# firstBusiness/mathmap

Hardware: AMD Instinct MI355X
Metric: Mpixels/sec (mandelbrot @8192x8192) (higher is better)
Workload: dtype f32

## Files before the change

### mathmap_amd/csrc/hipgen_internal.h

```cpp
#pragma once
#include <functional>
#include <memory>
#include <optional>
#include <ostream>
#include <string>
#include <vector>

#include "hipgen.h"

namespace mm {
namespace hipgen {

enum Slice { PROLOGUE, PIXEL, ROWS };

std::optional<int> env_int(const char *name);
struct Knobs {
    std::optional<int> unroll = env_int("MMHIP_UNROLL");
    std::optional<int> tile_w = env_int("MMHIP_TILE_W");
    std::optional<int> single_pixel = env_int("MMHIP_SINGLE_PIXEL");
    std::optional<int> pair = env_int("MMHIP_PAIR");
    bool pair_debug = env_int("MMHIP_PAIR_DEBUG").has_value();
    std::optional<int> pair_masks = env_int("MMHIP_PAIR_MASKS");
    std::optional<int> pair_exit = env_int("MMHIP_PAIR_EXIT");
    std::optional<int> pair_exit_tail = env_int("MMHIP_PAIR_EXIT_TAIL");
    std::optional<int> pair_pack = env_int("MMHIP_PAIR_PACK");
    std::optional<int> pair_peel = env_int("MMHIP_PAIR_PEEL");
    std::optional<int> pair_fma2 = env_int("MMHIP_PAIR_FMA2");
    bool pair_no_uniform = env_int("MMHIP_PAIR_NO_UNIFORM").has_value();
    std::optional<int> nt_store = env_int("MMHIP_NT_STORE");
    std::optional<int> xcd_order = env_int("MMHIP_XCD_ORDER");
    std::optional<int> waves_per_eu = env_int("MMHIP_WAVES_PER_EU");
    bool no_fetched_result = env_int("MMHIP_NO_FETCHED_RESULT").has_value();
    bool no_same_taps = env_int("MMHIP_NO_SAME_TAPS").has_value();
    bool no_outside_shortcut = env_int("MMHIP_NO_OUTSIDE_SHORTCUT").has_value();
    std::optional<int> frame_hot = env_int("MMHIP_FRAME_HOT");
    bool no_row_slice = env_int("MMHIP_NO_ROW_SLICE").has_value();
    std::optional<int> max_call_depth = env_int("MMHIP_MAX_CALL_DEPTH");
};

std::string vname(const Value *v);
std::string ctype(const CompVar *v);
int type_size(const CompVar *v);
std::string float_literal(float f);
const char *libm_name(const char *cname, bool f32);
bool is_truth_op(const char *cname);
bool is_pow2_divisor(float c);
bool nonneg_or_nan(const Value *v, int depth);
const Primary *sqrt_less_pow2(const Rhs &r, float *kk);

struct PairEnv {
    std::ostream &out;
    FilterCode &code;
    const KernelOptions &opt;
    const Knobs &knobs;
    const std::vector<Value *> &pix_defs;
    int pixel_stmts, pixel_fetches;
    std::function<std::string(const Primary &)> prim;
    std::function<std::string(const Stmt *)> rhs;
    std::function<bool(const Value *)> value_visible;
};
struct PairMode {
    virtual ~PairMode() {}
    virtual bool exit_driven() const = 0;
    virtual bool is_uniform(const Value *v) const = 0;
    virtual void emit_helpers() = 0;
    virtual void emit_pixel_loop(const std::string &ind) = 0;
};
std::unique_ptr<PairMode> make_pair_mode(const PairEnv &env);

}
}
```

### mathmap_amd/csrc/hipgen_pair.cpp

```cpp
#include <algorithm>
#include <cstdio>
#include <cstring>
#include <map>
#include <set>

#include "hipgen_internal.h"

namespace mm {
namespace hipgen {
namespace {

struct PairGen final : PairMode {
    PairEnv env;
    std::ostream &out;
    FilterCode &code;
    std::set<const Value *> defs;
    std::set<const Value *> bools;
    std::set<const Value *> uniform;
    int ids = 0;
    const bool exit = env.knobs.pair_exit.value_or(1) && env.knobs.pair_masks.value_or(1);
    const bool pack = exit && env.knobs.pair_pack.value_or(1);
    const Stmt *split_def = nullptr;
    bool split_leave = false;
    const bool fma2 = exit && env.knobs.pair_fma2.value_or(1) && env.knobs.pair_exit_tail.value_or(2) >= 2;
    struct Fuse { const Stmt *r, *d; Primary t, b; float k; bool keep_d; };
    std::map<const Stmt *, std::vector<Fuse>> fuse_plan;
    std::map<const Stmt *, const Fuse *> fusing;
    std::set<const Stmt *> fused_away;

    explicit PairGen(const PairEnv &e) : env(e), out(e.out), code(e.code) {}

    bool exit_driven() const override { return exit; }
    bool is_uniform(const Value *v) const override { return uniform.count(v) > 0; }

    static bool scalar_ty(Ty t) { return t == Ty::Int || t == Ty::Float; }
    static bool prim_ok(const Primary &p) {
        if (p.kind == Primary::IntConst || p.kind == Primary::FloatConst) return true;
        return p.kind == Primary::Val && scalar_ty(p.value->var->type);
    }
    static bool rhs_ok(const Rhs &r) {
        if (r.kind == Rhs::Prim) return prim_ok(r.prim);
        if (r.kind == Rhs::Internal) return r.internal == "x" || r.internal == "y";
        if (r.kind != Rhs::Op) return false;
        static const char *ok[] = {"ADD", "SUB", "MUL", "NEG", "DIV", "LESS", "LEQ", "EQ", "NOT", "sqrt"};
        bool found = false;
        for (const char *o : ok) found = found || !strcmp(r.op->cname, o);
        if (!found) return false;
        for (const Primary &a : r.args) if (!prim_ok(a)) return false;
        if (!strcmp(r.op->cname, "sqrt") && r.args[0].type() != Ty::Float) return false;
        if (!strcmp(r.op->cname, "NOT") && r.args[0].type() != Ty::Int) return false;
        return true;
    }
    bool block_ok(const Block &b) const {
        for (const Stmt *s : b) {
            if (!s->in_pixel) continue;
            switch (s->kind) {
                case Stmt::Assign:
                    if (!s->lhs || !scalar_ty(s->lhs->var->type) || !rhs_ok(s->rhs)) {
                        if (env.knobs.pair_debug)
                            fprintf(stderr, "pair mode: statement not covered (%s)\n",
                                    s->rhs.kind == Rhs::Op ? s->rhs.op->cname : s->rhs.kind == Rhs::Internal ? s->rhs.internal.c_str() : "rhs kind");
                        return false;
                    }
                    break;
                case Stmt::If:
                case Stmt::While:
                    if (s->cond.kind != Rhs::Prim || !prim_ok(s->cond.prim) || s->cond.prim.type() != Ty::Int) return false;
                    for (const Stmt *ph : s->phis) {
                        if (!ph->in_pixel) continue;
                        if (!scalar_ty(ph->lhs->var->type) || ph->rhs.kind != Rhs::Prim || ph->rhs2.kind != Rhs::Prim ||
                            !prim_ok(ph->rhs.prim) || !prim_ok(ph->rhs2.prim))
                            return false;
                    }
                    if (s->kind == Stmt::If ? !(block_ok(s->then_) && block_ok(s->else_)) : !block_ok(s->body)) return false;
                    break;
                default: break;
            }
        }
        return true;
    }
    bool eligible() const {
        if (!env.opt.fast_math_exact) return false;
        const bool force = env.knobs.pair.has_value();
        if (force && !*env.knobs.pair) return false;
        const int stmts = env.pixel_stmts;
        if (env.pixel_fetches || stmts < 4 || stmts > (force ? 400 : 40)) return false;
        const bool dbg = env.knobs.pair_debug;
        for (int i = 0; i < 4; ++i)
            if (!code.result[i] || !scalar_ty(code.result[i]->var->type)) {
                if (dbg) fprintf(stderr, "pair mode: result %d is not an int / float value\n", i);
                return false;
            }
        const bool ok = block_ok(code.body);
        if (dbg) fprintf(stderr, "pair mode: body %s (%d statements)\n", ok ? "covered" : "not covered", stmts);
        return ok;
    }

    template <class P> static bool truth_def(const Stmt *d, P operand) {
        if (d->kind == Stmt::Phi) return d->rhs.kind == Rhs::Prim && d->rhs2.kind == Rhs::Prim && operand(d->rhs.prim) && operand(d->rhs2.prim);
        if (d->kind != Stmt::Assign) return false;
        if (d->rhs.kind == Rhs::Prim) return operand(d->rhs.prim);
        return d->rhs.kind == Rhs::Op && is_truth_op(d->rhs.op->cname);
    }
    static bool const_is_bool(const Value *v, int depth) {
        if (!v || depth > 12 || v->var->type != Ty::Int) return false;
        if (v->index < 0) return true;
        return v->def && truth_def(v->def, [&](const Primary &p) {
            return p.kind == Primary::IntConst ? p.i == 0 || p.i == 1 : p.kind == Primary::Val && const_is_bool(p.value, depth + 1);
        });
    }
    bool prim_bool(const Primary &p) const {
        if (p.kind == Primary::IntConst) return p.i == 0 || p.i == 1;
        if (p.kind != Primary::Val) return false;
        if (p.value->index < 0) return p.value->var->type == Ty::Int;
        if (bools.count(p.value)) return true;
        return !defs.count(p.value) && const_is_bool(p.value, 0);
    }
    void infer_bools() {
        std::vector<const Stmt *> idefs;
        for (Value *v : env.pix_defs) {
            defs.insert(v);
            if (v->var->type == Ty::Int && v->def && v->def->lhs == v) idefs.push_back(v->def);
        }
        for (const Stmt *d : idefs) bools.insert(d->lhs);
        for (bool changed = true; changed;) {
            changed = false;
            for (const Stmt *d : idefs)
                if (bools.count(d->lhs) && !truth_def(d, [&](const Primary &p) { return prim_bool(p); })) { bools.erase(d->lhs); changed = true; }
        }
    }
    void uses_outside(const Block &b, const Stmt *skip, std::set<const Value *> &uses) const {
        auto use = [&](const Primary &p) { if (p.kind == Primary::Val) uses.insert(p.value); };
        auto use_rhs = [&](const Rhs &r) { if (r.kind == Rhs::Prim) use(r.prim); for (const Primary &a : r.args) use(a); };
        for (const Stmt *s : b) {
            if (!s->in_pixel) continue;
            if (s->kind == Stmt::Assign) use_rhs(s->rhs);
            if (s->kind == Stmt::If) {
                use_rhs(s->cond);
                uses_outside(s->then_, skip, uses);
                uses_outside(s->else_, skip, uses);
                for (const Stmt *ph : s->phis) if (ph->in_pixel) { use_rhs(ph->rhs); use_rhs(ph->rhs2); }
            }
            if (s->kind == Stmt::While) {
                for (const Stmt *ph : s->phis) if (ph->in_pixel) { use_rhs(ph->rhs); if (s != skip) use_rhs(ph->rhs2); }
                if (s != skip) { use_rhs(s->cond); uses_outside(s->body, skip, uses); }
            }
        }
    }

    std::string pbool(const Primary &p) {
        const std::string bu = exit ? "mm_xbu(" : "mm_bu(";
        if (p.kind == Primary::IntConst) return bu + (p.i ? "true)" : "false)");
        if (p.kind == Primary::Val && p.value->index < 0) return bu + "false)";
        if (uniform.count(p.value)) return "mm_bu((bool)u" + vname(p.value) + ")";
        if (bools.count(p.value)) return vname(p.value);
        return "mm_tob(" + pprim(p, Ty::Int) + ")";
    }
    std::string pprim(const Primary &p, Ty want) {
        const char *w = want == Ty::Float ? "mm_vf(" : "mm_vi(";
        if (p.kind == Primary::IntConst) return std::string(w) + std::to_string(p.i) + ")";
        if (p.kind == Primary::FloatConst) return std::string(w) + float_literal(p.f) + "f)";
        if (p.value->index < 0) return std::string(w) + "0)";
        if (uniform.count(p.value))
            return std::string(w) + (p.value->var->type == Ty::Float ? "(float)u" : "(int)u") + vname(p.value) + ")";
        return std::string(w) + vname(p.value) + ")";
    }
    static Ty arith_ty(const Rhs &r) {
        for (const Primary &a : r.args) if (a.type() == Ty::Float) return Ty::Float;
        return Ty::Int;
    }
    std::string prhs(const Rhs &r, const Value *lhs) {
        const Ty lhs_ty = lhs->var->type;
        const bool as_bool = bools.count(lhs) > 0;
        if (r.kind == Rhs::Prim) return as_bool ? pbool(r.prim) : pprim(r.prim, lhs_ty);
        if (r.kind == Rhs::Internal) return r.internal == "x" ? "mm_vf(x)" : "mm_y2";
        const char *cn = r.op->cname;
        const Ty t = arith_ty(r);
        const char *op = !strcmp(cn, "ADD") ? "+" : !strcmp(cn, "SUB") ? "-" : !strcmp(cn, "MUL") ? "*" : !strcmp(cn, "LESS") ? "<"
                         : !strcmp(cn, "LEQ") ? "<=" : !strcmp(cn, "EQ") ? "==" : nullptr;
        const bool compares = op && (op[0] == '<' || op[0] == '=');
        if (op && r.args.size() == 2 && ((r.args[0].type() == Ty::Int && r.args[1].kind == Primary::FloatConst) ||
                                         (r.args[1].type() == Ty::Int && r.args[0].kind == Primary::FloatConst))) {
            auto comp = [&](const Primary &p, const char *c) {
                if (p.kind == Primary::FloatConst) return "(double)" + float_literal(p.f) + "f";
                return "(double)" + pprim(p, Ty::Int) + "." + c;
            };
            const std::string ex = comp(r.args[0], "x") + " " + op + " " + comp(r.args[1], "x");
            const std::string ey = comp(r.args[0], "y") + " " + op + " " + comp(r.args[1], "y");
            if (compares) {
                const std::string b = "mm_bl(" + ex + ", " + ey + ")";
                return as_bool ? b : "mm_vi(" + b + ")";
            }
            return "mm_pf{(float)(" + ex + "), (float)(" + ey + ")}";
        }
        if (op && !compares) return "(" + pprim(r.args[0], t) + " " + op + " " + pprim(r.args[1], t) + ")";
        if (!strcmp(cn, "NEG")) return "(-" + pprim(r.args[0], t) + ")";
        if (!strcmp(cn, "sqrt")) return "mm_sqrt2(" + pprim(r.args[0], Ty::Float) + ")";
        if (!strcmp(cn, "DIV")) {
            if (r.args[1].kind == Primary::FloatConst || r.args[1].kind == Primary::IntConst) {
                const float c = r.args[1].kind == Primary::FloatConst ? r.args[1].f : (float)r.args[1].i;
                if (is_pow2_divisor(c)) return "(" + pprim(r.args[0], Ty::Float) + " * " + float_literal(1.0f / c) + "f)";
            }
            return "(" + pprim(r.args[0], Ty::Float) + " / " + pprim(r.args[1], Ty::Float) + ")";
        }
        std::string b;
        const std::string notb = exit ? "mm_xnotb(" : "mm_notb(";
        if (!strcmp(cn, "NOT")) b = notb + pbool(r.args[0]) + ")";
        else if (!strcmp(cn, "EQ") && prim_bool(r.args[0]) && prim_bool(r.args[1])) {
            const Primary &x = r.args[0], &y = r.args[1];
            if (y.kind == Primary::IntConst) b = y.i ? pbool(x) : notb + pbool(x) + ")";
            else if (x.kind == Primary::IntConst) b = x.i ? pbool(y) : notb + pbool(y) + ")";
            else b = "mm_eqb(" + pbool(x) + ", " + pbool(y) + ")";
        } else {
            float kk = 0;
            const Primary *sq = sqrt_less_pow2(r, &kk);
            if (sq && env.value_visible(sq->value)) {
                const std::string a = pprim(*sq, Ty::Float), k2 = "mm_vf(" + float_literal(kk) + "f)";
                b = nonneg_or_nan(sq->value, 0) ? "mm_lt(" + a + ", " + k2 + ")"
                                                : "mm_andb(mm_lt(" + a + ", " + k2 + "), mm_le(mm_vf(0.0f), " + a + "))";
            } else {
                const char *fn = !strcmp(cn, "LESS") ? "mm_lt(" : !strcmp(cn, "LEQ") ? "mm_le(" : "mm_eq(";
                b = fn + pprim(r.args[0], t) + ", " + pprim(r.args[1], t) + ")";
            }
        }
        return as_bool ? b : "mm_vi(" + b + ")";
    }
    std::string pair_ctype(const Value *v) const {
        return bools.count(v) ? "mm_bb" : v->var->type == Ty::Float ? "mm_pf" : "mm_pi";
    }
    std::string pval_as(const Primary &p, const Value *lhs) {
        return bools.count(lhs) ? pbool(p) : pprim(p, lhs->var->type);
    }

    bool invariant_scalar(const Primary &p) const {
        if (p.kind == Primary::IntConst || p.kind == Primary::FloatConst) return true;
        if (p.kind != Primary::Val) return false;
        return p.value->index < 0 || !defs.count(p.value);
    }
    bool uniform_operand(const Primary &p) const {
        return invariant_scalar(p) || (p.kind == Primary::Val && uniform.count(p.value));
    }
    void mark_uniform(const Block &b) {
        for (const Stmt *s : b) {
            if (!s->in_pixel) continue;
            if (s->kind == Stmt::Assign && s->rhs.kind != Rhs::Internal) {
                bool ok = s->rhs.kind == Rhs::Prim ? uniform_operand(s->rhs.prim) : s->rhs.kind == Rhs::Op;
                if (ok && s->rhs.kind == Rhs::Op)
                    for (const Primary &a : s->rhs.args) ok = ok && uniform_operand(a);
                if (ok && s->rhs.kind == Rhs::Prim && !(s->rhs.prim.kind == Primary::Val && uniform.count(s->rhs.prim.value))) ok = false;
                if (ok && bools.count(s->lhs) && !exit) ok = false;
                if (ok) uniform.insert(s->lhs);
            } else if (s->kind == Stmt::If) {
                mark_uniform(s->then_);
                mark_uniform(s->else_);
            }
        }
    }
    std::vector<const Stmt *> find_uniform_ivs(const Stmt *w) {
        std::vector<const Stmt *> ivs;
        if (env.knobs.pair_no_uniform) return ivs;
        for (const Stmt *ph : w->phis) {
            if (!ph->in_pixel || ph->rhs.kind != Rhs::Prim || ph->rhs2.kind != Rhs::Prim) continue;
            if (!scalar_ty(ph->lhs->var->type) || bools.count(ph->lhs)) continue;
            if (!invariant_scalar(ph->rhs.prim) || ph->rhs2.prim.kind != Primary::Val) continue;
            const Stmt *d = ph->rhs2.prim.value->def;
            if (!d || d->kind != Stmt::Assign || d->parent != w || d->rhs.kind != Rhs::Op || d->rhs.args.size() != 2) continue;
            const char *cn = d->rhs.op->cname;
            const Primary &a0 = d->rhs.args[0], &a1 = d->rhs.args[1];
            const bool self0 = a0.kind == Primary::Val && a0.value == ph->lhs, self1 = a1.kind == Primary::Val && a1.value == ph->lhs;
            const bool step = (!strcmp(cn, "ADD") && ((self0 && invariant_scalar(a1)) || (self1 && invariant_scalar(a0)))) ||
                              (!strcmp(cn, "SUB") && self0 && invariant_scalar(a1));
            if (!step) continue;
            ivs.push_back(ph);
            uniform.insert(ph->lhs);
        }
        if (!ivs.empty()) mark_uniform(w->body);
        return ivs;
    }

    struct Body {
        std::set<const Value *> defs;
        std::map<const Value *, const Stmt *> if_of;
        std::vector<const Stmt *> order;
        bool nested_loop = false;
    };
    void scan_body(const Block &b, Body &pb) const {
        for (const Stmt *s : b) {
            if (!s->in_pixel) continue;
            if (s->kind == Stmt::Assign) { pb.defs.insert(s->lhs); pb.order.push_back(s); }
            if (s->kind == Stmt::While) pb.nested_loop = true;
            if (s->kind == Stmt::If) {
                scan_body(s->then_, pb);
                scan_body(s->else_, pb);
                for (const Stmt *ph : s->phis)
                    if (ph->in_pixel) { pb.defs.insert(ph->lhs); pb.if_of[ph->lhs] = s; pb.order.push_back(ph); }
            }
        }
    }
    int eval3(const Primary &p, const Body &pb, const Value *l, int lv, int depth = 0) const {
        if (p.kind == Primary::IntConst) return p.i == 0 ? 0 : p.i == 1 ? 1 : -1;
        if (p.kind != Primary::Val || depth > 32) return -1;
        if (p.value->index < 0) return 0;
        if (p.value == l) return lv;
        if (!pb.defs.count(p.value) || !bools.count(p.value)) return -1;
        const Stmt *d = p.value->def;
        if (!d) return -1;
        if (d->kind == Stmt::Phi) {
            auto it = pb.if_of.find(p.value);
            if (it == pb.if_of.end() || d->rhs.kind != Rhs::Prim || d->rhs2.kind != Rhs::Prim) return -1;
            const Primary &cp = it->second->cond.prim;
            const int c = eval3(cp, pb, l, lv, depth + 1);
            const bool same1 = cp.kind == Primary::Val && d->rhs.prim.kind == Primary::Val && d->rhs.prim.value == cp.value && bools.count(cp.value);
            const bool same2 = cp.kind == Primary::Val && d->rhs2.prim.kind == Primary::Val && d->rhs2.prim.value == cp.value && bools.count(cp.value);
            const int a = same1 ? 1 : eval3(d->rhs.prim, pb, l, lv, depth + 1);
            const int b = same2 ? 0 : eval3(d->rhs2.prim, pb, l, lv, depth + 1);
            if (c == 1) return a;
            if (c == 0) return b;
            return a == b ? a : -1;
        }
        if (d->kind != Stmt::Assign) return -1;
        if (d->rhs.kind == Rhs::Prim) return eval3(d->rhs.prim, pb, l, lv, depth + 1);
        if (d->rhs.kind != Rhs::Op) return -1;
        const char *cn = d->rhs.op->cname;
        if (!strcmp(cn, "NOT")) { const int x = eval3(d->rhs.args[0], pb, l, lv, depth + 1); return x < 0 ? -1 : !x; }
        if (!strcmp(cn, "EQ") && prim_bool(d->rhs.args[0]) && prim_bool(d->rhs.args[1])) {
            const int x = eval3(d->rhs.args[0], pb, l, lv, depth + 1), y = eval3(d->rhs.args[1], pb, l, lv, depth + 1);
            return x < 0 || y < 0 ? -1 : x == y;
        }
        return -1;
    }
    const Stmt *find_split(const Stmt *w, const std::set<const Value *> &outside, bool &leave) const {
        if (w->cond.prim.kind != Primary::Val) return nullptr;
        Body pb;
        scan_body(w->body, pb);
        if (pb.nested_loop) return nullptr;
        const Stmt *cph = nullptr;
        for (const Stmt *ph : w->phis) if (ph->in_pixel && ph->lhs == w->cond.prim.value) cph = ph;
        if (!cph || cph->rhs2.kind != Rhs::Prim) return nullptr;
        for (const Stmt *d : pb.order) {
            if (d->kind != Stmt::Assign || !uniform.count(d->lhs) || !bools.count(d->lhs) || d->rhs.kind != Rhs::Op) continue;
            if (!is_truth_op(d->rhs.op->cname) || d->rhs.args.size() != 2) continue;
            if (d->rhs.args[0].type() != Ty::Int || d->rhs.args[1].type() != Ty::Int) continue;
            for (int lv = 0; lv < 2; ++lv) {
                if (eval3(cph->rhs2.prim, pb, d->lhs, lv) != 0) continue;
                std::set<const Value *> dep{d->lhs};
                auto in = [&](const Primary &p) { return p.kind == Primary::Val && dep.count(p.value) > 0; };
                for (const Stmt *q : pb.order) {
                    bool dp = false;
                    if (q->kind == Stmt::Assign) { if (q->rhs.kind == Rhs::Prim) dp = in(q->rhs.prim); for (const Primary &a : q->rhs.args) dp = dp || in(a); }
                    else dp = in(pb.if_of.at(q->lhs)->cond.prim) || in(q->rhs.prim) || in(q->rhs2.prim);
                    if (dp) dep.insert(q->lhs);
                }
                bool ok = true;
                for (const Stmt *ph : w->phis)
                    if (ph->in_pixel && outside.count(ph->lhs) && in(ph->rhs2.prim)) ok = false;
                if (!ok) continue;
                leave = lv != 0;
                return d;
            }
        }
        return nullptr;
    }
    bool tail_operand(const Primary &p, std::string &text, std::vector<std::string> &inputs, int first_input) {
        if (p.kind == Primary::IntConst) { text = std::to_string(p.i); return true; }
        if (p.kind != Primary::Val) return false;
        text = "%" + std::to_string(first_input + (int)inputs.size());
        inputs.push_back("__builtin_amdgcn_readfirstlane((int)(" + env.prim(p) + "))");
        return true;
    }

    struct Loop {
        Stmt *s;
        std::string ind, a;
        std::set<const Value *> outside;
        std::vector<const Stmt *> ivs;
        std::vector<std::pair<const Stmt *, std::string>> exit_copy;
        bool counted = false;
        unsigned count_step = 0;
        const Stmt *count_iv = nullptr;
        std::string count_twin;
        bool is_iv(const Stmt *ph) const { return std::find(ivs.begin(), ivs.end(), ph) != ivs.end(); }
    };
    void step_phis(const Loop &w, const std::string &I, bool select) {
        std::vector<Stmt *> phis;
        for (Stmt *ph : w.s->phis) if (ph->in_pixel && (select || !w.is_iv(ph))) phis.push_back(ph);
        for (size_t k = 0; k < phis.size(); ++k) {
            const std::string nv = pval_as(phis[k]->rhs2.prim, phis[k]->lhs);
            out << I << "const " << pair_ctype(phis[k]->lhs) << " " << w.a << "_n" << k << " = "
                << (select && w.outside.count(phis[k]->lhs) ? "mm_sel2(" + w.a + ", " + nv + ", " + vname(phis[k]->lhs) + ")" : nv) << ";\n";
        }
        for (size_t k = 0; k < phis.size(); ++k) out << I << vname(phis[k]->lhs) << " = " << w.a << "_n" << k << ";\n";
        for (const Stmt *ph : w.ivs)
            if (ph != w.count_iv) out << I << "u" << vname(ph->lhs) << " = " << env.prim(ph->rhs2.prim) << ";\n";
    }
    static bool counted_relation(const char *cn, bool leave, int side, long step, bool &inclusive) {
        if (!strcmp(cn, "EQ")) { inclusive = false; return leave && (step == 1 || step == -1); }
        const bool advancing_left = leave ? side == 1 : side == 0;
        inclusive = leave ? !strcmp(cn, "LESS") : !strcmp(cn, "LEQ");
        return advancing_left ? step > 0 : step < 0;
    }
    void plan_counted(Loop &w, const std::string &l) {
        if (env.knobs.pair_exit_tail.value_or(2) < 2) return;
        bool leave = false;
        const Stmt *split = find_split(w.s, w.outside, leave);
        if (!split) return;
        const char *cn = split->rhs.op->cname;
        const bool eq = !strcmp(cn, "EQ");
        int side = -1;
        const Stmt *iv = nullptr;
        long step = 0;
        bool stepped = false;
        for (int i = 0; i < 2 && side < 0; ++i) {
            const Primary &p = split->rhs.args[i];
            if (p.kind != Primary::Val) continue;
            for (const Stmt *ph : w.ivs) {
                if (ph->lhs->var->type != Ty::Int) continue;
                const Stmt *d = ph->rhs2.prim.value->def;
                const bool self0 = d->rhs.args[0].kind == Primary::Val && d->rhs.args[0].value == ph->lhs;
                const Primary &c = d->rhs.args[self0 ? 1 : 0];
                if (c.kind != Primary::IntConst || (p.value != ph->lhs && p.value != d->lhs)) continue;
                side = i; iv = ph; stepped = p.value == d->lhs;
                step = !strcmp(d->rhs.op->cname, "SUB") ? -(long)c.i : (long)c.i;
            }
        }
        if (side < 0 || step == 0 || step > 0x7fffffffL || step < -0x7fffffffL) return;
        const Primary &bound = split->rhs.args[1 - side], &init = iv->rhs.prim;
        if (!invariant_scalar(bound) || bound.type() != Ty::Int || init.type() != Ty::Int) return;
        bool inclusive = false;
        if (!counted_relation(cn, leave, side, step, inclusive)) return;
        const bool up = step > 0;
        const long pre = stepped ? 0 : -step;
        auto lit = [](const Primary &p, long &v) {
            if (p.kind == Primary::IntConst) { v = p.i; return true; }
            if (p.kind == Primary::Val && p.value->index < 0) { v = 0; return true; }
            return false;
        };
        long iv0 = 0, b0 = 0;
        const std::string k = l + "_k";
        if (lit(init, iv0) && lit(bound, b0)) {
            long d = up ? b0 - (iv0 + pre) : (iv0 + pre) - b0;
            if (eq) d &= 0xffffffffL; else d += inclusive ? 1 : 0;
            if (!eq && d > 0xffffffffL) return;
            const bool exact = eq || d > 0;
            if (!exact) d = 1;
            const unsigned k0 = 0u - (unsigned)d;
            out << w.ind << "unsigned " << k << " = " << k0 << "u;\n";
            if (exact) {
                w.count_iv = iv;
                const unsigned c = up ? (unsigned)iv0 - k0 : (unsigned)iv0 + k0;
                w.count_twin = "(int)(" + std::to_string(c) + "u " + (up ? "+ " : "- ") + k + ")";
            }
        } else {
            uniform.erase(iv->lhs);
            const std::string o = "((long)(" + env.prim(init) + ") + " + std::to_string(pre) + "l)", b = "(long)(" + env.prim(bound) + ")";
            uniform.insert(iv->lhs);
            const std::string d = (up ? b + " - " + o : o + " - " + b) + (inclusive ? " + 1l" : "");
            out << w.ind << "const long " << k << "_d = " << d << ";\n";
            out << w.ind << "unsigned " << k << " = __builtin_amdgcn_readfirstlane(0u - (unsigned)("
                << (eq ? k + "_d" : k + "_d <= 0l ? 1l : " + k + "_d > 0xffffffffl ? 0xffffffffl : " + k + "_d") << "));\n";
        }
        w.counted = true;
        w.count_step = (unsigned)(up ? step : -step);
    }
    void selecting_iteration(const Loop &w) {
        Stmt *s = w.s;
        const std::string &ind = w.ind, &a = w.a;
        stmts(s->body, ind + "  ", a);
        step_phis(w, ind + "  ", true);
        out << ind << "  " << a << " = mm_andb(" << a << ", " << pbool(s->cond.prim) << ");\n";
    }
    void exit_driven_iteration(const Loop &w, const std::string &l) {
        Stmt *s = w.s;
        const std::string &ind = w.ind, &a = w.a, I2 = ind + "    ";
        bool leave = false;
        const Stmt *split = find_split(s, w.outside, leave);
        std::vector<std::string> tail_inputs;
        std::string tail_o0, tail_o1;
        const bool asm_tail = split && !w.counted && env.knobs.pair_exit_tail.value_or(1) &&
                              !(split->rhs.args[0].kind == Primary::IntConst && split->rhs.args[1].kind == Primary::IntConst) &&
                              tail_operand(split->rhs.args[0], tail_o0, tail_inputs, 8) && tail_operand(split->rhs.args[1], tail_o1, tail_inputs, 8);
        out << ind << "  mm_bb " << l << ";"
            << (w.counted ? " unsigned long " + l + "_t;" : asm_tail ? " unsigned long " + l + "_u, " + l + "_t;" : split ? " bool " + l + "_b;" : "") << "\n";
        out << ind << "  do {\n";
        if (w.count_iv) out << I2 << "const int u" << vname(w.count_iv->lhs) << " = " << w.count_twin << ";\n";
        const Stmt *outer_split = split_def;
        const bool outer_leave = split_leave;
        split_def = split;
        split_leave = leave;
        stmts(s->body, I2, a);
        split_def = outer_split;
        split_leave = outer_leave;
        if (asm_tail)
            for (size_t i = 0; i < tail_inputs.size(); ++i) {
                out << I2 << "const int " << l << "_o" << i << " = " << tail_inputs[i] << ";\n";
                tail_inputs[i] = l + "_o" + std::to_string(i);
            }
        else if (split && !w.counted)
            out << I2 << l << "_b = (bool)(" << env.rhs(split) << ") == " << (leave ? "true" : "false") << ";\n";
        step_phis(w, I2, false);
        const std::string c = pbool(s->cond.prim);
        const std::string lx = a + ".x & ~" + c + ".x", ly = a + ".y & ~" + c + ".y";
        if (w.counted) {
            out << I2 << "const mm_bb " << l << "_c = " << c << ";\n";
            out << I2 << "asm(\"s_andn2_b64 %0, %4, %6\\n\\ts_andn2_b64 %1, %5, %7\\n\\ts_or_b64 %3, %0, %1\\n\\ts_add_u32 %2, %2, " << w.count_step
                << "\\n\\ts_cselect_b64 %3, -1, %3\"\n"
                << I2 << "    : \"=&s\"(" << l << ".x), \"=&s\"(" << l << ".y), \"+s\"(" << l << "_k), \"=&s\"(" << l << "_t)\n"
                << I2 << "    : \"s\"(" << a << ".x), \"s\"(" << a << ".y), \"s\"(" << l << "_c.x), \"s\"(" << l << "_c.y) : \"scc\");\n";
            out << ind << "  } while (" << l << "_t == 0);\n";
            out << ind << "  if (" << l << "_k < " << w.count_step << "u) " << l << " = " << a << ";      // the counter has wrapped: every active lane leaves\n";
            if (w.count_iv) out << ind << "  u" << vname(w.count_iv->lhs) << " = " << w.count_twin << ";\n";
        } else if (asm_tail) {
            const char *cn = split->rhs.op->cname;
            const char *cmp = !strcmp(cn, "LESS") ? "s_cmp_lt_i32" : !strcmp(cn, "LEQ") ? "s_cmp_le_i32" : "s_cmp_eq_i32";
            out << I2 << "const mm_bb " << l << "_c = " << c << ";\n";
            out << I2 << "asm(\"" << cmp << " " << tail_o0 << ", " << tail_o1 << "\\n\\ts_cselect_b64 %2, " << (leave ? "-1, 0" : "0, -1")
                << "\\n\\ts_andn2_b64 %0, %4, %6\\n\\ts_andn2_b64 %1, %5, %7\\n\\ts_or_b64 %3, %2, %0\\n\\ts_or_b64 %3, %3, %1\"\n"
                << I2 << "    : \"=&s\"(" << l << ".x), \"=&s\"(" << l << ".y), \"=&s\"(" << l << "_u), \"=&s\"(" << l << "_t)\n"
                << I2 << "    : \"s\"(" << a << ".x), \"s\"(" << a << ".y), \"s\"(" << l << "_c.x), \"s\"(" << l << "_c.y)";
            for (const std::string &in : tail_inputs) out << ", \"s\"(" << in << ")";
            out << " : \"scc\");\n";
            out << ind << "  } while (" << l << "_t == 0);\n";
            out << ind << "  " << l << ".x |= " << a << ".x & " << l << "_u; " << l << ".y |= " << a << ".y & " << l << "_u;\n";
        } else if (split) {
            out << I2 << l << " = mm_bb{" << lx << ", " << ly << "};\n";
            out << ind << "  } while (!" << l << "_b && (" << l << ".x | " << l << ".y) == 0);\n";
            out << ind << "  if (" << l << "_b) " << l << " = " << a << ";      // the uniform conjunct has ended the loop: every active lane leaves\n";
        } else {
            out << I2 << l << " = mm_bb{" << lx << ", " << ly << "};\n";
            out << ind << "  } while ((" << l << ".x | " << l << ".y) == 0);\n";
        }
        for (const auto &e : w.exit_copy) {
            std::string nv = vname(e.first->lhs);
            if (w.is_iv(e.first)) nv = e.first->lhs->var->type == Ty::Float ? "mm_vf((float)u" + nv + ")" : "mm_vi(mm_s2v((int)u" + nv + "))";
            out << ind << "  " << e.second << " = mm_sel2(" << l << ", " << nv << ", " << e.second << ");\n";
        }
        out << ind << "  " << a << ".x &= ~" << l << ".x; " << a << ".y &= ~" << l << ".y;\n";
    }
    struct Uses { std::map<const Value *, int> live, dead; };
    template <class F> static void each_phi(const Block &b, F f) {
        for (const Stmt *s : b) {
            for (const Stmt *ph : s->phis) f(ph);
            each_phi(s->then_, f);
            each_phi(s->else_, f);
            each_phi(s->body, f);
        }
    }
    static void count_roots(const Block &b, std::map<const Value *, int> &n) {
        auto use = [&](const Primary &p) { if (p.kind == Primary::Val) ++n[p.value]; };
        auto use_rhs = [&](const Rhs &r) { if (r.kind == Rhs::Prim) use(r.prim); for (const Primary &a : r.args) use(a); };
        for (const Stmt *s : b) {
            if (s->kind == Stmt::Assign) use_rhs(s->rhs);
            if (s->kind == Stmt::If || s->kind == Stmt::While) use_rhs(s->cond);
            count_roots(s->then_, n);
            count_roots(s->else_, n);
            count_roots(s->body, n);
        }
    }
    Uses count_uses() const {
        Uses u;
        count_roots(code.body, u.live);
        for (int i = 0; i < 4; ++i) if (code.result[i]) ++u.live[code.result[i]];
        std::vector<const Stmt *> phis;
        each_phi(code.body, [&](const Stmt *ph) { phis.push_back(ph); });
        std::set<const Stmt *> live_phis;
        auto operands = [](const Stmt *ph, auto f) {
            for (const Rhs *r : {&ph->rhs, &ph->rhs2}) if (r->kind == Rhs::Prim && r->prim.kind == Primary::Val) f(r->prim.value);
        };
        for (bool changed = true; changed;) {
            changed = false;
            for (const Stmt *ph : phis)
                if (!live_phis.count(ph) && u.live.count(ph->lhs)) {
                    live_phis.insert(ph);
                    operands(ph, [&](const Value *v) { ++u.live[v]; });
                    changed = true;
                }
        }
        for (const Stmt *ph : phis)
            if (!live_phis.count(ph)) operands(ph, [&](const Value *v) { ++u.dead[v]; });
        return u;
    }
    static void defined_in(const Block &b, std::set<const Value *> &d) {
        for (const Stmt *s : b) {
            if (s->kind == Stmt::Assign) d.insert(s->lhs);
            for (const Stmt *ph : s->phis) d.insert(ph->lhs);
            defined_in(s->then_, d);
            defined_in(s->else_, d);
            defined_in(s->body, d);
        }
    }
    static int count_stmts(const Block &b) {
        int n = 0;
        for (const Stmt *s : b)
            if (s->in_pixel) n += 1 + count_stmts(s->then_) + count_stmts(s->else_) + count_stmts(s->body);
        return n;
    }
    static bool pow2_multiplier(const Primary &p, float &k) {
        if (p.kind != Primary::IntConst && p.kind != Primary::FloatConst) return false;
        k = p.kind == Primary::IntConst ? (float)p.i : p.f;
        if (!(k >= 2.0f) || k > 0x1p127f) return false;
        unsigned bits;
        memcpy(&bits, &k, 4);
        return (bits & 0x7fffffu) == 0;
    }
    static bool doubling(const Stmt *d, Primary &t, float &k) {
        if (d->kind != Stmt::Assign || !d->in_pixel || d->lhs->var->type != Ty::Float || d->rhs.kind != Rhs::Op || d->rhs.args.size() != 2) return false;
        const Primary &a0 = d->rhs.args[0], &a1 = d->rhs.args[1];
        auto fval = [](const Primary &p) { return p.kind == Primary::Val && p.value->var->type == Ty::Float; };
        if (!strcmp(d->rhs.op->cname, "ADD") && fval(a0) && fval(a1) && a0.value == a1.value) { t = a0; k = 2.0f; return true; }
        if (strcmp(d->rhs.op->cname, "MUL")) return false;
        if (fval(a0) && pow2_multiplier(a1, k)) { t = a0; return true; }
        if (fval(a1) && pow2_multiplier(a0, k)) { t = a1; return true; }
        return false;
    }
    void plan_block(const Block &b, const std::set<const Value *> &in_loop, const Uses &uses, std::vector<Fuse> &fs) const {
        for (const Stmt *r : b) {
            if (!r->in_pixel) continue;
            if (r->kind == Stmt::If) { plan_block(r->then_, in_loop, uses, fs); plan_block(r->else_, in_loop, uses, fs); }
            if (r->kind != Stmt::Assign || r->lhs->var->type != Ty::Float || uniform.count(r->lhs)) continue;
            if (r->rhs.kind != Rhs::Op || strcmp(r->rhs.op->cname, "ADD") || r->rhs.args.size() != 2) continue;
            for (int i = 0; i < 2; ++i) {
                const Primary &dp = r->rhs.args[i], &bp = r->rhs.args[1 - i];
                if (dp.kind != Primary::Val || dp.value->index < 0 || !dp.value->def || dp.value->def->lhs != dp.value) continue;
                const Stmt *d = dp.value->def;
                Fuse f{r, d, Primary(), bp, 0.0f, uses.dead.count(d->lhs) > 0};
                if (std::find(b.begin(), b.end(), d) == b.end() || uniform.count(d->lhs) || !doubling(d, f.t, f.k)) continue;
                const auto n = uses.live.find(d->lhs);
                if (n == uses.live.end() || n->second != 1) continue;
                if (bp.kind == Primary::FloatConst) { if (!(__builtin_fabsf(bp.f) <= 0x1p102f)) continue; }
                else if (bp.kind == Primary::Val) { if (bp.value->var->type != Ty::Float || in_loop.count(bp.value)) continue; }
                else if (bp.kind != Primary::IntConst) continue;
                fs.push_back(f);
                break;
            }
        }
    }
    void plan_loops(const Block &b, const Uses &uses) {
        for (const Stmt *s : b) {
            if (!s->in_pixel) continue;
            if (s->kind == Stmt::If) { plan_loops(s->then_, uses); plan_loops(s->else_, uses); }
            if (s->kind != Stmt::While) continue;
            const std::vector<const Stmt *> ivs = find_uniform_ivs(s);
            std::set<const Value *> in_loop;
            for (const Stmt *ph : s->phis) in_loop.insert(ph->lhs);
            defined_in(s->body, in_loop);
            std::vector<Fuse> fs;
            plan_block(s->body, in_loop, uses, fs);
            const bool guarded = std::any_of(fs.begin(), fs.end(), [&](const Fuse &f) { return needs_guard(f.b); });
            if (!fs.empty() && (!guarded || 2 * count_stmts(s->body) <= (env.knobs.pair.has_value() ? 400 : 40))) fuse_plan[s] = fs;
            plan_loops(s->body, uses);
            for (const Stmt *ph : ivs) uniform.erase(ph->lhs);
        }
    }
    void plan_fusion() {
        if (!fma2) return;
        const Uses uses = count_uses();
        const std::set<const Value *> keep = uniform;
        plan_loops(code.body, uses);
        uniform = keep;
    }
    static bool needs_guard(const Primary &b) { return b.kind == Primary::Val && b.value->index >= 0; }
    void fused_loop(const Loop &w, const std::vector<Fuse> &fs, const std::string &id, const std::string &mask) {
        const std::string &ind = w.ind, I1 = ind + "  ";
        std::vector<std::string> addends;
        for (const Fuse &f : fs) {
            if (!needs_guard(f.b)) continue;
            const std::string b = pprim(f.b, Ty::Float);
            if (std::find(addends.begin(), addends.end(), b) == addends.end()) addends.push_back(b);
        }
        auto copy = [&](bool fused, const std::string &l, const std::string &I) {
            Loop c = w;
            c.ind = I;
            if (fused) for (const Fuse &f : fs) { fusing[f.r] = &f; if (!f.keep_d) fused_away.insert(f.d); }
            plan_counted(c, l);
            out << I << "while (" << c.a << ".x | " << c.a << ".y) {\n";
            exit_driven_iteration(c, l);
            out << I << "}\n";
            if (fused) for (const Fuse &f : fs) { fusing.erase(f.r); fused_away.erase(f.d); }
        };
        out << ind << "mm_bb " << w.a << " = mm_andb(" << mask << ", " << pbool(w.s->cond.prim) << ");\n";
        if (addends.empty()) { copy(true, "mm_l" + id, ind); return; }
        out << ind << "const bool mm_g" << id << " = ";
        for (size_t i = 0; i < addends.size(); ++i) out << (i ? " && " : "") << "mm_fma2_ok(" << addends[i] << ")";
        out << ";\n" << ind << "if (!mm_g" << id << ") {\n";
        copy(false, "mm_l" + id, I1);
        out << ind << "} else {\n";
        copy(true, "mm_l" + std::to_string(ids++), I1);
        out << ind << "}\n";
    }
    void while_loop(Stmt *s, const std::string &ind, const std::string &mask) {
        const std::string id = std::to_string(ids++);
        Loop w{s, ind, "mm_a" + id, {}, {}, {}};
        uses_outside(code.body, s, w.outside);
        for (int i = 0; i < 4; ++i) w.outside.insert(code.result[i]);
        if (!exit && s->cond.prim.kind == Primary::Val) w.outside.insert(s->cond.prim.value);
        for (Stmt *ph : s->phis)
            if (ph->in_pixel) out << ind << vname(ph->lhs) << " = " << pval_as(ph->rhs.prim, ph->lhs) << ";\n";
        if (exit) {
            int k = 0;
            for (Stmt *ph : s->phis) {
                if (!ph->in_pixel) continue;
                if (w.outside.count(ph->lhs)) w.exit_copy.push_back({ph, w.a + "_e" + std::to_string(k)});
                ++k;
            }
            for (const auto &e : w.exit_copy) out << ind << pair_ctype(e.first->lhs) << " " << e.second << " = " << vname(e.first->lhs) << ";\n";
        }
        w.ivs = find_uniform_ivs(s);
        for (const Stmt *ph : w.ivs) {
            uniform.erase(ph->lhs);
            const std::string init = env.prim(ph->rhs.prim);
            uniform.insert(ph->lhs);
            out << ind << (ph->lhs->var->type == Ty::Float ? "float u" : "int u") << vname(ph->lhs) << " = " << init << ";\n";
        }
        const auto fp = fuse_plan.find(s);
        if (fp != fuse_plan.end()) fused_loop(w, fp->second, id, mask);
        else {
            if (exit) plan_counted(w, "mm_l" + id);
            out << ind << "mm_bb " << w.a << " = mm_andb(" << mask << ", " << pbool(s->cond.prim) << ");\n";
            out << ind << "while (" << w.a << ".x | " << w.a << ".y) {\n";
            if (exit) exit_driven_iteration(w, "mm_l" + id);
            else selecting_iteration(w);
            out << ind << "}\n";
        }
        for (const auto &e : w.exit_copy) out << ind << vname(e.first->lhs) << " = " << e.second << ";\n";
        for (const Stmt *ph : w.ivs) uniform.erase(ph->lhs);
    }

    void stmts(Block &b, const std::string &ind, const std::string &mask) {
        for (Stmt *s : b) {
            if (!s->in_pixel) continue;
            switch (s->kind) {
                case Stmt::Assign:
                    if (s == split_def) {
                        out << ind << "const bool u" << vname(s->lhs) << " = " << (split_leave ? "false" : "true") << ";\n";
                        break;
                    }
                    if (uniform.count(s->lhs)) {
                        const char *ty = bools.count(s->lhs) ? "bool" : s->lhs->var->type == Ty::Float ? "float" : "int";
                        out << ind << "const " << ty << " u" << vname(s->lhs) << " = " << env.rhs(s) << ";\n";
                        break;
                    }
                    if (fused_away.count(s)) break;
                    if (fusing.count(s)) {
                        const Fuse &f = *fusing.at(s);
                        const std::string t = pprim(f.t, Ty::Float), k = float_literal(f.k) + "f", b = pprim(f.b, Ty::Float);
                        out << ind << vname(s->lhs) << " = mm_pf{__builtin_fmaf(" << t << ".x, " << k << ", " << b << ".x), __builtin_fmaf("
                            << t << ".y, " << k << ", " << b << ".y)};\n";
                        break;
                    }
                    out << ind << vname(s->lhs) << " = " << prhs(s->rhs, s->lhs) << ";\n";
                    break;
                case Stmt::If: {
                    const std::string c = "mm_c" + std::to_string(ids++);
                    out << ind << "const mm_bb " << c << " = " << pbool(s->cond.prim) << ";\n";
                    stmts(s->then_, ind, "mm_andb(" + mask + ", " + c + ")");
                    stmts(s->else_, ind, "mm_andb(" + mask + (exit ? ", mm_xnotb(" : ", mm_notb(") + c + "))");
                    for (Stmt *ph : s->phis)
                        if (ph->in_pixel)
                            out << ind << vname(ph->lhs) << " = mm_sel2(" << c << ", " << pval_as(ph->rhs.prim, ph->lhs) << ", "
                                << pval_as(ph->rhs2.prim, ph->lhs) << ");\n";
                    break;
                }
                case Stmt::While: while_loop(s, ind, mask); break;
                default: break;
            }
        }
    }

    void emit_helpers() override {
        if (exit)
            out << R"(#define MM_PAIR_EXIT 1
// exit-driven pair loops (hipgen.cpp pair_while_exit).  mm_xnotb: a lane mask's bits outside exec are never read -- selects
// read their own lane's bit, and every mask a branch tests is ANDed with one that lies inside exec -- so NOT needs no re-AND
// and a broadcast no ballot.
MM_DEV mm_bb mm_xnotb(mm_bb a) { return mm_bb{~a.x, ~a.y}; }
MM_DEV mm_bb mm_xbu(bool u) { const unsigned long m = u ? ~0ul : 0ul; return mm_bb{m, m}; }      // a literal truth value, likewise
// a wave-uniform int for the exit copies, moved from its scalar register where it is wanted (as an ordinary operand it
// would pull the loop counter, and the loop's bound test, onto the vector unit)
MM_DEV int mm_s2v(int u) { int r; asm("v_mov_b32 %0, %1" : "=v"(r) : "s"(__builtin_amdgcn_readfirstlane(u))); return r; }
)";
        bool guarded = false;
        for (const auto &lp : fuse_plan) for (const Fuse &f : lp.second) guarded = guarded || needs_guard(f.b);
        if (guarded)
            out << R"(#define MM_PAIR_FMA2 1
// fused doubling (hipgen_pair.cpp plan_fusion): fl(fl(t * 2^k) + b) is fma(t, 2^k, b) -- the product is exact -- unless the
// product overflows and the exact sum does not, which takes |b| > 2^103.  True when no lane of the wave holds such an
// addend in either pixel (NaN fails the comparison): the loop then runs in its fused copy.
MM_DEV bool mm_fma2_ok(mm_pf b) {
  return __builtin_amdgcn_ballot_w64(!(__builtin_fabsf(b.x) <= 0x1p102f && __builtin_fabsf(b.y) <= 0x1p102f)) == 0ul;
}
)";
        emit_store_pair();
    }

    struct Pack {
        std::vector<const Value *> vals;
        int src[4];
        float lit[4];
    };
    static bool literal_of(const Value *v, float &f, int depth = 0) {
        if (!v || depth > 8) return false;
        if (v->index < 0) { f = 0; return true; }
        const Stmt *d = v->def;
        if (!d || d->kind != Stmt::Assign || d->lhs != v || d->rhs.kind != Rhs::Prim) return false;
        const Primary &p = d->rhs.prim;
        if (p.kind == Primary::IntConst) { f = (float)p.i; return true; }
        if (p.kind == Primary::FloatConst) { f = p.f; return v->var->type == Ty::Float && f == f; }
        return p.kind == Primary::Val && p.value->var->type == v->var->type && literal_of(p.value, f, depth + 1);
    }
    bool plan_pack(Pack &pk) const {
        if (!pack) return false;
        for (int i = 0; i < 4; ++i) {
            const Value *v = code.result[i];
            pk.src[i] = -1;
            if (literal_of(v, pk.lit[i])) continue;
            const auto it = std::find(pk.vals.begin(), pk.vals.end(), v);
            pk.src[i] = (int)(it - pk.vals.begin());
            if (it == pk.vals.end()) pk.vals.push_back(v);
        }
        return !pk.vals.empty();
    }
    void emit_store_pair() {
        Pack pk;
        if (!plan_pack(pk)) return;
        const int n = (int)pk.vals.size();
        unsigned k = 0;
        for (int i = 0; i < 4; ++i)
            if (pk.src[i] < 0) {
                const float c = pk.lit[i] < 0.0f ? 0.0f : pk.lit[i] > 1.0f ? 1.0f : pk.lit[i];
                k |= (unsigned)(255.0 * (double)c) << (8 * i);
            }
        auto sel = [&](int second, int first) {
            unsigned s = 0;
            for (int i = 0; i < 4; ++i) s |= (pk.src[i] == second && second >= 0 ? 0x00u : pk.src[i] == first && first >= 0 ? 0x04u : 0x0cu) << (8 * i);
            return s;
        };
        auto hex = [](unsigned v) { char b[16]; snprintf(b, sizeof b, "0x%08xu", v); return std::string(b); };
        auto word = [&](const char *px) {
            auto u = [&](int j) { return std::string("u") + px + std::to_string(j); };
            if (n == 1) {
                unsigned s1 = 0;
                for (int i = 0; i < 4; ++i) s1 |= (pk.src[i] == 0 ? 0x04u : (unsigned)i) << (8 * i);
                return "__builtin_amdgcn_perm(" + u(0) + ", " + hex(k) + ", " + hex(s1) + ")";
            }
            std::string w = "__builtin_amdgcn_perm(" + u(1) + ", " + u(0) + ", " + hex(sel(0, 1)) + ")";
            if (n > 2) w += " | __builtin_amdgcn_perm(" + (n > 3 ? u(3) : u(2)) + ", " + u(2) + ", " + hex(sel(2, n > 3 ? 3 : -1)) + ")";
            return k ? w + " | " + hex(k) : w;
        };
        out << "// this kernel's result pack (hipgen_pair.cpp emit_store_pair): both pixels of a step, " << n << " distinct value" << (n > 1 ? "s" : "")
            << " per pixel, literal bytes " << hex(k) << "\n"
            << "MM_DEV void mm_store_pair(const mm_args &A, int row_a, int row_b, int col";
        for (int j = 0; j < n; ++j) out << ", float a" << j << ", float b" << j;
        out << ") {\n  if (__builtin_expect(!A.floatmap && A.output_bpp == 4, 1)) {\n   ";
        for (int j = 0; j < n; ++j) out << " a" << j << " = mm_clamp01(a" << j << "); b" << j << " = mm_clamp01(b" << j << ");";
        out << "\n    unsigned";
        for (int j = 0; j < n; ++j) out << (j ? ", " : " ") << "ua" << j << ", ub" << j;
        out << ";\n    asm volatile(\"s_setreg_imm32_b32 hwreg(HW_REG_MODE, 0, 2), 3\\n\\t\"\n";
        for (int j = 0; j < 2 * n; ++j) out << "                 \"v_fma_f32 %" << j << ", %" << 2 * n + j << ", %" << 4 * n << ", %" << 4 * n + 1 << "\\n\\t\"\n";
        out << "                 \"s_setreg_imm32_b32 hwreg(HW_REG_MODE, 0, 2), 0\"\n                 :";
        for (int j = 0; j < n; ++j) out << (j ? ", " : " ") << "\"=&v\"(ua" << j << "), \"=&v\"(ub" << j << ")";
        out << "\n                 :";
        for (int j = 0; j < n; ++j) out << " \"v\"(a" << j << "), \"v\"(b" << j << "),";
        out << " \"s\"(255.0f), \"v\"(8388608.0f));\n"
            << "    MM_STORE_U32((unsigned *)((unsigned char *)A.out + (long)row_a * A.row_stride + (long)col * 4), " << word("a") << ");\n"
            << "    MM_STORE_U32((unsigned *)((unsigned char *)A.out + (long)row_b * A.row_stride + (long)col * 4), " << word("b") << ");\n"
            << "    return;\n  }\n  mm_tup<4> ra, rb;\n";
        for (int i = 0; i < 4; ++i) {
            if (pk.src[i] < 0) out << "  ra.v[" << i << "] = rb.v[" << i << "] = " << float_literal(pk.lit[i]) << "f;\n";
            else out << "  ra.v[" << i << "] = a" << pk.src[i] << "; rb.v[" << i << "] = b" << pk.src[i] << ";\n";
        }
        out << "  mm_store_pixel(A, row_a, col, ra);\n  mm_store_pixel(A, row_b, col, rb);\n}\n";
    }
    void emit_pixel_loop(const std::string &I) override {
        out << "#pragma unroll 1\n" << I << "for (; mm_p < A.ppt; mm_p += 2) {\n"
            << I << "  // vertically adjacent pixels: they mostly take the same path (a wave covers 16 x 8 pixels per step)\n"
            << I << "  const int rl_a = row0 + (int)(threadIdx.x / MM_TILE_W) + mm_p * MM_TILE_H, rl_b = rl_a + 1;\n"
            << I << "  const int row_a = rl_a < A.num_rows ? rl_a : A.num_rows - 1, row_b = rl_b < A.num_rows ? rl_b : A.num_rows - 1;\n"
            << I << "  const mm_pf mm_y2 = {A.ytab[row_a], A.ytab[row_b]};    // CALC_VIRTUAL_Y per row, by the prologue\n";
        std::set<Value *> seen;
        for (Value *v : env.pix_defs)
            if (v->index >= 0 && seen.insert(v).second) out << I << "  " << pair_ctype(v) << " " << vname(v) << ";\n";
        stmts(code.body, I + "  ", "mm_bu(true)");
        Pack pk;
        if (plan_pack(pk)) {
            out << I << "  // a row past the end was evaluated as the last row: storing it there again writes the same bytes\n"
                << I << "  mm_store_pair(A, row_a, row_b, col";
            for (const Value *v : pk.vals) {
                const std::string e = pprim(Primary::V(const_cast<Value *>(v)), Ty::Float);
                out << ", " << e << ".x, " << e << ".y";
            }
            out << ");\n" << I << "}\n";
            return;
        }
        out << I << "  mm_tup<4> mm_ra, mm_rb;\n";
        for (int i = 0; i < 4; ++i) {
            const std::string v = pprim(Primary::V(code.result[i]), Ty::Float);
            out << I << "  mm_ra.v[" << i << "] = " << v << ".x; mm_rb.v[" << i << "] = " << v << ".y;\n";
        }
        out << I << "  // a row past the end was evaluated as the last row: storing it there again writes the same bytes\n"
            << I << "  mm_store_pixel(A, row_a, col, mm_ra);\n"
            << I << "  mm_store_pixel(A, row_b, col, mm_rb);\n" << I << "}\n";
    }
};

}

std::unique_ptr<PairMode> make_pair_mode(const PairEnv &env) {
    std::unique_ptr<PairGen> g(new PairGen(env));
    if (!g->eligible()) return nullptr;
    g->infer_bools();
    g->plan_fusion();
    return g;
}

}
}
```

Measured before the change: 425,800.

## Hoist wave-uniform checks out of paired pixel loop onto scalar unit

Adds a default-on 'step' mode to the paired-pixel HIP generator. Truth values defined outside the loop are read once per work-item via readfirstlane and kept in SGPRs as lane masks. The store fast-path test is precomputed into one wave-uniform flag, with 32-bit address arithmetic when the bounds allow it. The counted-loop wrap fixup uses scalar select asm, and empty asm pins the entry masks in SGPRs. The aim is to cut per-iteration VALU and scalar overhead, at the cost of more inline asm and register constraints that could hurt scheduling.

```diff
diff --git a/mathmap_amd/csrc/hipgen_internal.h b/mathmap_amd/csrc/hipgen_internal.h
--- a/mathmap_amd/csrc/hipgen_internal.h
+++ b/mathmap_amd/csrc/hipgen_internal.h
@@ -26,6 +26,7 @@
     std::optional<int> pair_pack = env_int("MMHIP_PAIR_PACK");
     std::optional<int> pair_peel = env_int("MMHIP_PAIR_PEEL");
     std::optional<int> pair_fma2 = env_int("MMHIP_PAIR_FMA2");
+    std::optional<int> pair_step = env_int("MMHIP_PAIR_STEP");
     bool pair_no_uniform = env_int("MMHIP_PAIR_NO_UNIFORM").has_value();
     std::optional<int> nt_store = env_int("MMHIP_NT_STORE");
     std::optional<int> xcd_order = env_int("MMHIP_XCD_ORDER");
diff --git a/mathmap_amd/csrc/hipgen_pair.cpp b/mathmap_amd/csrc/hipgen_pair.cpp
--- a/mathmap_amd/csrc/hipgen_pair.cpp
+++ b/mathmap_amd/csrc/hipgen_pair.cpp
@@ -3,6 +3,7 @@
 #include <cstring>
 #include <map>
 #include <set>
+#include <sstream>
 
 #include "hipgen_internal.h"
 
@@ -27,6 +28,8 @@
     std::map<const Stmt *, std::vector<Fuse>> fuse_plan;
     std::map<const Stmt *, const Fuse *> fusing;
     std::set<const Stmt *> fused_away;
+    bool step = false;
+    std::vector<const Value *> step_truths;
 
     explicit PairGen(const PairEnv &e) : env(e), out(e.out), code(e.code) {}
 
@@ -154,6 +157,10 @@
         if (p.kind == Primary::Val && p.value->index < 0) return bu + "false)";
         if (uniform.count(p.value)) return "mm_bu((bool)u" + vname(p.value) + ")";
         if (bools.count(p.value)) return vname(p.value);
+        if (step && !defs.count(p.value)) {
+            if (std::find(step_truths.begin(), step_truths.end(), p.value) == step_truths.end()) step_truths.push_back(p.value);
+            return "mm_bb{mm_t_" + vname(p.value) + ", mm_t_" + vname(p.value) + "}";
+        }
         return "mm_tob(" + pprim(p, Ty::Int) + ")";
     }
     std::string pprim(const Primary &p, Ty want) {
@@ -507,7 +514,11 @@
                 << I2 << "    : \"=&s\"(" << l << ".x), \"=&s\"(" << l << ".y), \"+s\"(" << l << "_k), \"=&s\"(" << l << "_t)\n"
                 << I2 << "    : \"s\"(" << a << ".x), \"s\"(" << a << ".y), \"s\"(" << l << "_c.x), \"s\"(" << l << "_c.y) : \"scc\");\n";
             out << ind << "  } while (" << l << "_t == 0);\n";
-            out << ind << "  if (" << l << "_k < " << w.count_step << "u) " << l << " = " << a << ";      // the counter has wrapped: every active lane leaves\n";
+            if (step)
+                out << ind << "  { unsigned " << l << "_w; asm(\"s_sub_u32 %2, %3, " << w.count_step << "\\n\\ts_cselect_b64 %0, %4, %0\\n\\ts_cselect_b64 %1, %5, %1\" : \"+s\"(" << l
+                    << ".x), \"+s\"(" << l << ".y), \"=&s\"(" << l << "_w) : \"s\"(" << l << "_k), \"s\"(" << a << ".x), \"s\"(" << a << ".y) : \"scc\"); }\n";
+            else
+                out << ind << "  if (" << l << "_k < " << w.count_step << "u) " << l << " = " << a << ";      // the counter has wrapped: every active lane leaves\n";
             if (w.count_iv) out << ind << "  u" << vname(w.count_iv->lhs) << " = " << w.count_twin << ";\n";
         } else if (asm_tail) {
             const char *cn = split->rhs.op->cname;
@@ -652,11 +663,14 @@
         }
     }
     void plan_fusion() {
-        if (!fma2) return;
+        if (!exit || env.knobs.pair_exit_tail.value_or(2) < 2) return;
         const Uses uses = count_uses();
         const std::set<const Value *> keep = uniform;
         plan_loops(code.body, uses);
         uniform = keep;
+        const bool fuses = !fuse_plan.empty();
+        if (!fma2) fuse_plan.clear();
+        step = pack && env.knobs.pair_step.value_or(1) && (fma2 || !fuses);
     }
     static bool needs_guard(const Primary &b) { return b.kind == Primary::Val && b.value->index >= 0; }
     void fused_loop(const Loop &w, const std::vector<Fuse> &fs, const std::string &id, const std::string &mask) {
@@ -672,6 +686,7 @@
             c.ind = I;
             if (fused) for (const Fuse &f : fs) { fusing[f.r] = &f; if (!f.keep_d) fused_away.insert(f.d); }
             plan_counted(c, l);
+            entry_mask(c, I);
             out << I << "while (" << c.a << ".x | " << c.a << ".y) {\n";
             exit_driven_iteration(c, l);
             out << I << "}\n";
@@ -687,6 +702,9 @@
         copy(true, "mm_l" + std::to_string(ids++), I1);
         out << ind << "}\n";
     }
+    void entry_mask(const Loop &w, const std::string &I) {
+        if (step) out << I << "asm(\"\" : \"+s\"(" << w.a << ".x), \"+s\"(" << w.a << ".y));\n";
+    }
     void while_loop(Stmt *s, const std::string &ind, const std::string &mask) {
         const std::string id = std::to_string(ids++);
         Loop w{s, ind, "mm_a" + id, {}, {}, {}};
@@ -716,6 +734,7 @@
         else {
             if (exit) plan_counted(w, "mm_l" + id);
             out << ind << "mm_bb " << w.a << " = mm_andb(" << mask << ", " << pbool(s->cond.prim) << ");\n";
+            if (exit) entry_mask(w, ind);
             out << ind << "while (" << w.a << ".x | " << w.a << ".y) {\n";
             if (exit) exit_driven_iteration(w, "mm_l" + id);
             else selecting_iteration(w);
@@ -850,7 +869,8 @@
             << " per pixel, literal bytes " << hex(k) << "\n"
             << "MM_DEV void mm_store_pair(const mm_args &A, int row_a, int row_b, int col";
         for (int j = 0; j < n; ++j) out << ", float a" << j << ", float b" << j;
-        out << ") {\n  if (__builtin_expect(!A.floatmap && A.output_bpp == 4, 1)) {\n   ";
+        if (step) out << ", unsigned mm_s32) {\n  if (__builtin_expect(mm_s32 != 0u, 1)) {\n   ";
+        else out << ") {\n  if (__builtin_expect(!A.floatmap && A.output_bpp == 4, 1)) {\n   ";
         for (int j = 0; j < n; ++j) out << " a" << j << " = mm_clamp01(a" << j << "); b" << j << " = mm_clamp01(b" << j << ");";
         out << "\n    unsigned";
         for (int j = 0; j < n; ++j) out << (j ? ", " : " ") << "ua" << j << ", ub" << j;
@@ -860,10 +880,14 @@
         for (int j = 0; j < n; ++j) out << (j ? ", " : " ") << "\"=&v\"(ua" << j << "), \"=&v\"(ub" << j << ")";
         out << "\n                 :";
         for (int j = 0; j < n; ++j) out << " \"v\"(a" << j << "), \"v\"(b" << j << "),";
-        out << " \"s\"(255.0f), \"v\"(8388608.0f));\n"
-            << "    MM_STORE_U32((unsigned *)((unsigned char *)A.out + (long)row_a * A.row_stride + (long)col * 4), " << word("a") << ");\n"
-            << "    MM_STORE_U32((unsigned *)((unsigned char *)A.out + (long)row_b * A.row_stride + (long)col * 4), " << word("b") << ");\n"
-            << "    return;\n  }\n  mm_tup<4> ra, rb;\n";
+        out << " \"s\"(255.0f), \"v\"(8388608.0f));\n";
+        for (const char *px : {"a", "b"})
+            if (step)
+                out << "    MM_STORE_U32((unsigned *)((unsigned char *)A.out + (((unsigned)row_" << px
+                    << " & 0xffffffu) * ((unsigned)A.row_stride & 0xffffffu) + (unsigned)col * 4u)), " << word(px) << ");\n";
+            else
+                out << "    MM_STORE_U32((unsigned *)((unsigned char *)A.out + (long)row_" << px << " * A.row_stride + (long)col * 4), " << word(px) << ");\n";
+        out << "    return;\n  }\n  mm_tup<4> ra, rb;\n";
         for (int i = 0; i < 4; ++i) {
             if (pk.src[i] < 0) out << "  ra.v[" << i << "] = rb.v[" << i << "] = " << float_literal(pk.lit[i]) << "f;\n";
             else out << "  ra.v[" << i << "] = a" << pk.src[i] << "; rb.v[" << i << "] = b" << pk.src[i] << ";\n";
@@ -871,6 +895,25 @@
         out << "  mm_store_pixel(A, row_a, col, ra);\n  mm_store_pixel(A, row_b, col, rb);\n}\n";
     }
     void emit_pixel_loop(const std::string &I) override {
+        Pack lean;
+        if (step && plan_pack(lean)) {
+            std::ostringstream body;
+            std::streambuf *const sb = out.rdbuf(body.rdbuf());
+            emit_pixel_loop_text(I, true);
+            out.rdbuf(sb);
+            out << I << "// once per work-item (hipgen_pair.cpp emit_pixel_loop): wave-uniform, on the scalar unit\n";
+            for (const Value *v : step_truths)
+                out << I << "unsigned mm_w_" << vname(v) << " = __builtin_amdgcn_readfirstlane(" << vname(v) << " != 0 ? ~0u : 0u);\n"
+                    << I << "asm(\"\" : \"+s\"(mm_w_" << vname(v) << "));\n"
+                    << I << "const unsigned long mm_t_" << vname(v) << " = ((unsigned long)mm_w_" << vname(v) << " << 32) | mm_w_" << vname(v) << ";\n";
+            out << I << "unsigned mm_s32 = __builtin_amdgcn_readfirstlane((unsigned)(!A.floatmap && A.output_bpp == 4 && A.row_stride >= 0 && A.row_stride < (1 << 24) &&\n"
+                << I << "    A.num_rows <= (1 << 24) && (unsigned long)(unsigned)(A.num_rows - 1) * (unsigned)A.row_stride + (unsigned long)(unsigned)A.region_width * 4ul <= 0xfffffffful));\n"
+                << body.str();
+            return;
+        }
+        emit_pixel_loop_text(I, false);
+    }
+    void emit_pixel_loop_text(const std::string &I, bool lean) {
         out << "#pragma unroll 1\n" << I << "for (; mm_p < A.ppt; mm_p += 2) {\n"
             << I << "  // vertically adjacent pixels: they mostly take the same path (a wave covers 16 x 8 pixels per step)\n"
             << I << "  const int rl_a = row0 + (int)(threadIdx.x / MM_TILE_W) + mm_p * MM_TILE_H, rl_b = rl_a + 1;\n"
@@ -883,12 +926,13 @@
         Pack pk;
         if (plan_pack(pk)) {
             out << I << "  // a row past the end was evaluated as the last row: storing it there again writes the same bytes\n"
+                << (lean ? I + "  asm(\"\" : \"+s\"(mm_s32));\n" : "")
                 << I << "  mm_store_pair(A, row_a, row_b, col";
             for (const Value *v : pk.vals) {
                 const std::string e = pprim(Primary::V(const_cast<Value *>(v)), Ty::Float);
                 out << ", " << e << ".x, " << e << ".y";
             }
-            out << ");\n" << I << "}\n";
+            out << (lean ? ", mm_s32);\n" : ");\n") << I << "}\n";
             return;
         }
         out << I << "  mm_tup<4> mm_ra, mm_rb;\n";
```

Measured after the change: 428,500 (median of 6 runs). Within noise of the previous version (+0.6%).
